# 0xMiden/miden-vm

Measured on NVIDIA H100. Metric: trace cells/sec proved, higher is better.
Workload: dtype u64

## Files before the change

### miden-vm_b200/csrc/kernels.cu

```cuda
#include "kernels.cuh"
#include "poseidon2.cuh"
#include "poseidon2_fast2.cuh"
#include "ntt2.cuh"
#include "blake3.cuh"
#include "keccak.cuh"
#include "rescue.cuh"
#include <algorithm>
#include <cstdio>

namespace mk {

static unsigned long long g_launches = 0;
unsigned long long launch_count() { return g_launches; }
void count_launch() { ++g_launches; }
void reset_launch_count() { g_launches = 0; }
#define COUNT_LAUNCH() (++g_launches)

void upload_constants() {
    cudaMemcpyToSymbol(p2::D_RC_EXT_INITIAL, p2::P2_RC_EXT_INITIAL, sizeof(u64) * 48);
    cudaMemcpyToSymbol(p2::D_RC_INTERNAL, p2::P2_RC_INTERNAL, sizeof(u64) * 22);
    cudaMemcpyToSymbol(p2::D_RC_EXT_TERMINAL, p2::P2_RC_EXT_TERMINAL, sizeof(u64) * 48);
    cudaMemcpyToSymbol(rsc::D_ARK1, rsc::RESCUE_ARK1, sizeof(u64) * 84);
    cudaMemcpyToSymbol(rsc::D_ARK2, rsc::RESCUE_ARK2, sizeof(u64) * 84);
}

#ifdef MDN_EMULATED
static inline void st_release_sys(u64* p, u64 v) { __atomic_store_n(p, v, __ATOMIC_RELEASE); }
static inline u64 ld_acquire_sys(const u64* p) { return __atomic_load_n(p, __ATOMIC_ACQUIRE); }
static constexpr long long BARRIER_TIMEOUT = 600ll * 1000000000ll;
#else
__device__ __forceinline__ void st_release_sys(u64* p, u64 v) { asm volatile("st.release.sys.global.u64 [%0], %1;" ::"l"(p), "l"(v) : "memory"); }
__device__ __forceinline__ u64 ld_acquire_sys(const u64* p) { u64 v; asm volatile("ld.acquire.sys.global.u64 %0, [%1];" : "=l"(v) : "l"(p) : "memory"); return v; }
static constexpr long long BARRIER_TIMEOUT = 30000000000ll;
#endif
__device__ __forceinline__ void push_u2(const PushDst& d, size_t idx, size_t owner_key, ulonglong2 v) {
    if (d.mode == PUSH_ALL) {
        for (u32 g = 0; g < d.world; g++) reinterpret_cast<ulonglong2*>(d.pp.p[g])[idx] = v;
    } else {
        u32 g = d.mode == PUSH_OWNER ? (u32)(owner_key >> d.owner_shift) : d.rank;
        reinterpret_cast<ulonglong2*>(d.pp.p[g])[idx] = v;
    }
}
struct BarrierArgs { PeerPtrs flags; u32 rank, world; u64 epoch; u32* err; };
__global__ void k_barrier(BarrierArgs a) {
    u32 p = threadIdx.x;
    if (p < a.world) { __threadfence_system(); st_release_sys(a.flags.p[p] + a.rank, a.epoch); }
    __syncthreads();
    if (p < a.world) {
        long long t0 = clock64();
        while (ld_acquire_sys(a.flags.p[a.rank] + p) < a.epoch) {
            if (clock64() - t0 > BARRIER_TIMEOUT) { atomicOr(a.err, 8u); break; }
#ifdef MDN_EMULATED
            emu::cpu_relax();
#endif
        }
    }
}
void launch_barrier(const PeerPtrs& flags, u32 rank, u32 world, u64 epoch, u32* err, cudaStream_t st) {
    BarrierArgs a; a.flags = flags; a.rank = rank; a.world = world; a.epoch = epoch; a.err = err;
    k_barrier<<<1, 32, 0, st>>>(a);
    COUNT_LAUNCH();
}
struct PushArgs { const u64* src; PeerPtrs dst; u32 rank, world; size_t n; };
__global__ void __launch_bounds__(256) k_push(PushArgs a) {
    size_t stride = (size_t)gridDim.x * blockDim.x, i0 = (size_t)blockIdx.x * blockDim.x + threadIdx.x;
    if ((a.n & 1) == 0 && (((size_t)a.src) & 15) == 0) {
        const ulonglong2* s2 = reinterpret_cast<const ulonglong2*>(a.src);
        for (size_t i = i0; i < a.n / 2; i += stride) {
            ulonglong2 v = s2[i];
            for (u32 g = 0; g < a.world; g++) if (g != a.rank) reinterpret_cast<ulonglong2*>(a.dst.p[g])[i] = v;
        }
    } else {
        for (size_t i = i0; i < a.n; i += stride) {
            u64 v = a.src[i];
            for (u32 g = 0; g < a.world; g++) if (g != a.rank) a.dst.p[g][i] = v;
        }
    }
}
void launch_push(const u64* src, const PeerPtrs& dst, u32 rank, u32 world, size_t n, cudaStream_t st) {
    if (!n || world <= 1) return;
    PushArgs a; a.src = src; a.dst = dst; a.rank = rank; a.world = world; a.n = n;
    unsigned blocks = (unsigned)std::min<size_t>((n / 2 + 255) / 256 + 1, 132 * 8);
    k_push<<<blocks, 256, 0, st>>>(a);
    COUNT_LAUNCH();
}

struct TransposeDst { PeerPtrs dst; PeerPtrs bad; u32 world; };
__global__ void k_transpose(const u64* __restrict__ src, TransposeDst d, u32 n_rows, u32 width, size_t col_stride, u32 row0) {
    __shared__ u64 tile[32][33];
    u32 r0 = blockIdx.x * 32, c0 = blockIdx.y * 32;
    bool any_bad = false;
    for (u32 i = threadIdx.y; i < 32; i += 8) {
        u32 r = r0 + i, c = c0 + threadIdx.x;
        if (r < n_rows && c < width) {
            u64 v = src[(size_t)r * width + c];
            any_bad |= (v >= gl::P);
            tile[i][threadIdx.x] = v;
        }
    }
    if (any_bad) for (u32 g = 0; g < d.world; g++) if (d.bad.p[g]) atomicOr(reinterpret_cast<u32*>(d.bad.p[g]), 1u);
    __syncthreads();
    for (u32 i = threadIdx.y; i < 32; i += 8) {
        u32 c = c0 + i, r = r0 + threadIdx.x;
        if (r < n_rows && c < width) {
            u64 v = tile[threadIdx.x][i];
            size_t o = (size_t)c * col_stride + row0 + r;
            for (u32 g = 0; g < d.world; g++) d.dst.p[g][o] = v;
        }
    }
}
void launch_transpose_rm_to_cm(const u64* src, u64* dst, u32 n_rows, u32 width, u32* d_bad_flag, cudaStream_t st) {
    TransposeDst d{}; d.dst.p[0] = dst; d.bad.p[0] = reinterpret_cast<u64*>(d_bad_flag); d.world = 1;
    dim3 grid((n_rows + 31) / 32, (width + 31) / 32), block(32, 8);
    k_transpose<<<grid, block, 0, st>>>(src, d, n_rows, width, (size_t)n_rows, 0u);
    COUNT_LAUNCH();
}
void launch_transpose_slice_push(const u64* src_slice, const PeerPtrs& dst_cm, const PeerPtrs& bad, u32 world, u32 row0, u32 n_rows_slice,
                                 u32 n_rows_total, u32 width, cudaStream_t st) {
    if (!n_rows_slice || !width) return;
    TransposeDst d{}; d.dst = dst_cm; d.bad = bad; d.world = world;
    dim3 grid((n_rows_slice + 31) / 32, (width + 31) / 32), block(32, 8);
    k_transpose<<<grid, block, 0, st>>>(src_slice, d, n_rows_slice, width, (size_t)n_rows_total, row0);
    COUNT_LAUNCH();
}

__global__ void __launch_bounds__(256) k_ingest_cm(const u64* __restrict__ src, u64* __restrict__ dst, size_t n, u32* bad) {
    const bool store = src != dst;
    size_t stride = (size_t)gridDim.x * blockDim.x, i0 = (size_t)blockIdx.x * blockDim.x + threadIdx.x;
    bool any_bad = false;
    if (((((size_t)src) | ((size_t)dst)) & 15) == 0) {
        const ulonglong2* s2 = reinterpret_cast<const ulonglong2*>(src);
        ulonglong2* d2 = reinterpret_cast<ulonglong2*>(dst);
        for (size_t i = i0; i < n / 2; i += stride) {
            ulonglong2 v = s2[i];
            any_bad |= (v.x >= gl::P) | (v.y >= gl::P);
            if (store) d2[i] = v;
        }
        if ((n & 1) && i0 == 0) {
            u64 v = src[n - 1];
            any_bad |= v >= gl::P;
            if (store) dst[n - 1] = v;
        }
    } else {
        for (size_t i = i0; i < n; i += stride) {
            u64 v = src[i];
            any_bad |= v >= gl::P;
            if (store) dst[i] = v;
        }
    }
    if (any_bad) atomicOr(bad, 1u);
}
void launch_ingest_cm(const u64* src_cm, u64* dst_cm, size_t n, u32* d_bad_flag, cudaStream_t st) {
    if (!n) return;
    unsigned blocks = (unsigned)std::min<size_t>((n / 2 + 255) / 256 + 1, 132 * 8);
    k_ingest_cm<<<blocks, 256, 0, st>>>(src_cm, dst_cm, n, d_bad_flag);
    COUNT_LAUNCH();
}

static constexpr int NTT_THREADS = 256;
static inline unsigned ntt_threads(u32 m, u32 log_cols, u32 log_elems) {
    u32 g = (m + log_cols >= log_elems) ? (1u << (m + log_cols - log_elems)) : 1u;
    if (g < 32) g = 32;
    if (g > 256) g = 256;
    return g;
}

__device__ __forceinline__ u64 w_pow(const u64* __restrict__ hi, const u64* __restrict__ lo, u32 lo_bits, u64 e) {
    return gl::mul(hi[e >> lo_bits], lo[e & ((1ull << lo_bits) - 1)]);
}

#define NTT_BOUNDS __launch_bounds__(NTT_THREADS)
template <int N1C, int N2C>
__global__ void NTT_BOUNDS k_intt_strided(u64* cols, size_t col_stride, NttTables T, u32 log_c) {
    extern __shared__ u64 sm[];
    ntt2::intt_strided_block<N1C, N2C>(blockIdx.x, blockIdx.y, sm, cols, col_stride, T, log_c);
}
template <int N2C>
__global__ void NTT_BOUNDS k_intt_contig(u64* cols, size_t col_stride, NttTables T) {
    extern __shared__ u64 sm[];
    ntt2::intt_contig_block<N2C>(blockIdx.x, blockIdx.y, sm, cols, col_stride, T);
}
template <int N1C, int N2C>
__global__ void NTT_BOUNDS k_fwd_contig(const FwdItem* __restrict__ items, NttTables T, PremulTables Pm) {
    extern __shared__ u64 sm[];
    ntt2::fwd_contig_block<N1C, N2C>(blockIdx.x, blockIdx.y, sm, items, T, Pm);
}
template <int N1C, int N2C>
__global__ void NTT_BOUNDS k_fwd_strided(const FwdItem* __restrict__ items, NttTables T, u32 log_c) {
    extern __shared__ u64 sm[];
    ntt2::fwd_strided_block<N1C, N2C>(blockIdx.x, blockIdx.y, sm, items, T, log_c);
}
#define NTT_SPECIALISED(X) X(8, 8) X(8, 9) X(9, 9) X(9, 10) X(10, 10) X(10, 11) X(11, 11)

template <int N1C, int N2C>
static void launch_intt_t(u64* cols, size_t col_stride, u32 n_cols, const NttTables& T, u32 log_c, cudaStream_t st) {
    u32 N1 = 1u << T.n1, N2 = 1u << T.n2, C = 1u << log_c;
    constexpr u32 LOG_E1 = N1C >= 0 ? ntt2::sched_log_elems(N1C) : 3, LOG_E2 = N2C >= 0 ? ntt2::sched_log_elems(N2C) : 3;
    if (T.n1 > 0) {
        size_t smem = ntt2::smem_words_strided(T.n1, log_c) * sizeof(u64);
        cudaFuncSetAttribute(k_intt_strided<N1C, N2C>, cudaFuncAttributeMaxDynamicSharedMemorySize, (int)smem);
        k_intt_strided<N1C, N2C><<<dim3(N2 / C, n_cols), ntt_threads(T.n1, log_c, LOG_E1), smem, st>>>(cols, col_stride, T, log_c);
        COUNT_LAUNCH();
    }
    size_t smem = ntt2::smem_words_contig_inv(T.n2) * sizeof(u64);
    k_intt_contig<N2C><<<dim3(N1, n_cols), ntt_threads(T.n2, 0, LOG_E2), smem, st>>>(cols, col_stride, T);
    COUNT_LAUNCH();
}
void launch_intt(u64* cols, size_t col_stride, u32 n_cols, const NttTables& T, cudaStream_t st) {
    u32 log_c = T.n1 >= 12 ? 0 : 12 - T.n1; if (log_c > T.n2) log_c = T.n2;
#define X(a, b) if (T.n1 == a && T.n2 == b) { launch_intt_t<a, b>(cols, col_stride, n_cols, T, log_c, st); return; }
    NTT_SPECIALISED(X)
#undef X
    launch_intt_t<-1, -1>(cols, col_stride, n_cols, T, log_c, st);
}
template <int N1C, int N2C>
static void launch_fwd_t(const FwdItem* d_items, u32 n_items, const NttTables& T, const PremulTables& Pm, u32 log_c, cudaStream_t st) {
    u32 N1 = 1u << T.n1, N2 = 1u << T.n2, C = 1u << log_c;
    constexpr u32 LOG_E1 = N1C >= 0 ? ntt2::sched_log_elems(N1C) : 3, LOG_E2 = N2C >= 0 ? ntt2::sched_log_elems(N2C) : 3;
    size_t smem = ntt2::smem_words_contig_fwd(T.n2) * sizeof(u64);
    k_fwd_contig<N1C, N2C><<<dim3(N1, n_items), ntt_threads(T.n2, 0, LOG_E2), smem, st>>>(d_items, T, Pm);
    COUNT_LAUNCH();
    if (T.n1 > 0) {
        size_t smem2 = ntt2::smem_words_strided(T.n1, log_c) * sizeof(u64);
        cudaFuncSetAttribute(k_fwd_strided<N1C, N2C>, cudaFuncAttributeMaxDynamicSharedMemorySize, (int)smem2);
        k_fwd_strided<N1C, N2C><<<dim3(N2 / C, n_items), ntt_threads(T.n1, log_c, LOG_E1), smem2, st>>>(d_items, T, log_c);
        COUNT_LAUNCH();
    }
}
void launch_fwd_ntt(const FwdItem* d_items, u32 n_items, const NttTables& T, const PremulTables& Pm, cudaStream_t st) {
    u32 log_c = T.n1 >= 12 ? 0 : 12 - T.n1; if (log_c > T.n2) log_c = T.n2;
#define X(a, b) if (T.n1 == a && T.n2 == b) { launch_fwd_t<a, b>(d_items, n_items, T, Pm, log_c, st); return; }
    NTT_SPECIALISED(X)
#undef X
    launch_fwd_t<-1, -1>(d_items, n_items, T, Pm, log_c, st);
}

static constexpr int HASH_THREADS = 128;
static constexpr int HASH_MIN_BLOCKS = 6;

enum { PERM_P2 = 0, PERM_RPO = 3, PERM_RPX = 4 };
template <int PERM>
__device__ __forceinline__ void alg_permute(u64* s) {
    if constexpr (PERM == PERM_RPO) rsc::rpo_permute(s);
    else if constexpr (PERM == PERM_RPX) rsc::rpx_permute(s);
    else p2f::permute(s);
}
#define ALG_BOUNDS(PERM) __launch_bounds__(HASH_THREADS, (PERM) == PERM_P2 ? HASH_MIN_BLOCKS : 1)
#define ALG_DISPATCH(perm, CALL) do { if ((perm) == PERM_RPO) { CALL(PERM_RPO); } else if ((perm) == PERM_RPX) { CALL(PERM_RPX); } else { CALL(PERM_P2); } } while (0)

template <int PERM>
__global__ void ALG_BOUNDS(PERM) k_leaf_hash(LeafArgs a, u32 log_n, u32 log_b, const u64* __restrict__ prev,
                                                            u32 prev_log_n, u64* __restrict__ states_out,
                                                            PushDst dig, u32 has_dig, u32 t0, u32 nt) {
    size_t L = (size_t)1 << (log_n + log_b);
    size_t idx = (size_t)blockIdx.x * blockDim.x + threadIdx.x;
    if (idx >= ((size_t)nt << log_n)) return;
    u32 t = t0 + (u32)(idx >> log_n);
    u32 r = (u32)(idx & (((size_t)1 << log_n) - 1));
    size_t pos = ((size_t)t << log_n) + r;
    u64 s[12];
    if (prev) {
        size_t Lp = (size_t)1 << (prev_log_n + log_b);
        size_t pp = ((size_t)t << prev_log_n) + (r & ((1u << prev_log_n) - 1));
#pragma unroll
        for (int k = 0; k < 12; k++) s[k] = prev[k * Lp + pp];
    } else {
#pragma unroll
        for (int k = 0; k < 12; k++) s[k] = 0;
    }
    for (int m = 0; m < a.n_mats; m++) {
        const u64* base = a.m[m].base + pos;
        u32 w = a.m[m].width;
        for (u32 c0 = 0; c0 < w; c0 += 8) {
#pragma unroll
            for (u32 k = 0; k < 8; k++) s[k] = (c0 + k < w) ? base[(size_t)(c0 + k) * L] : 0ull;
            alg_permute<PERM>(s);
        }
    }
    if (states_out) {
#pragma unroll
        for (int k = 0; k < 12; k++) states_out[k * L + pos] = glf::canon(s[k]);
    }
    if (has_dig) {
        size_t i = ((size_t)r << log_b) | t;
        push_u2(dig, 2 * i, i, make_ulonglong2(glf::canon(s[0]), glf::canon(s[1])));
        push_u2(dig, 2 * i + 1, i, make_ulonglong2(glf::canon(s[2]), glf::canon(s[3])));
    }
}
template <int PERM>
static void launch_leaf_hash_t(const LeafArgs& a, u32 log_n, u32 log_blowup, const u64* prev_states, u32 prev_log_n,
                               u64* states_out, const PushDst* dig, u32 t0, u32 nt, cudaStream_t st) {
    size_t cnt = (size_t)nt << log_n;
    unsigned blocks = (unsigned)((cnt + HASH_THREADS - 1) / HASH_THREADS);
    PushDst d = dig ? *dig : local_dst(nullptr);
    k_leaf_hash<PERM><<<blocks, HASH_THREADS, 0, st>>>(a, log_n, log_blowup, prev_states, prev_log_n, states_out, d, dig ? 1u : 0u, t0, nt);
    COUNT_LAUNCH();
}
void launch_leaf_hash(const LeafArgs& a, u32 log_n, u32 log_blowup, const u64* prev_states, u32 prev_log_n,
                      u64* states_out, const PushDst* dig, u32 t0, u32 nt, cudaStream_t st, int perm) {
#define X(PM) launch_leaf_hash_t<PM>(a, log_n, log_blowup, prev_states, prev_log_n, states_out, dig, t0, nt, st)
    ALG_DISPATCH(perm, X);
#undef X
}

template <int PERM>
__global__ void ALG_BOUNDS(PERM) k_compress(const u64* __restrict__ ch, u64* __restrict__ par, size_t n) {
    size_t i = (size_t)blockIdx.x * blockDim.x + threadIdx.x;
    if (i >= n) return;
    const ulonglong2* c = reinterpret_cast<const ulonglong2*>(ch + i * 8);
    ulonglong2 a0 = c[0], a1 = c[1], b0 = c[2], b1 = c[3];
    u64 s[12] = {a0.x, a0.y, a1.x, a1.y, b0.x, b0.y, b1.x, b1.y, 0, 0, 0, 0};
    alg_permute<PERM>(s);
    ulonglong2* d = reinterpret_cast<ulonglong2*>(par + i * 4);
    d[0] = make_ulonglong2(glf::canon(s[0]), glf::canon(s[1]));
    d[1] = make_ulonglong2(glf::canon(s[2]), glf::canon(s[3]));
}
template <int PERM>
static void launch_compress_layer_t(const u64* children, u64* parents, size_t n_parents, cudaStream_t st) {
    unsigned blocks = (unsigned)((n_parents + HASH_THREADS - 1) / HASH_THREADS);
    k_compress<PERM><<<blocks, HASH_THREADS, 0, st>>>(children, parents, n_parents);
    COUNT_LAUNCH();
}
void launch_compress_layer(const u64* children, u64* parents, size_t n_parents, cudaStream_t st, int perm) {
#define X(PM) launch_compress_layer_t<PM>(children, parents, n_parents, st)
    ALG_DISPATCH(perm, X);
#undef X
}

template <int PERM>
__global__ void __launch_bounds__(HASH_THREADS) k_fri_leaf(const u64* __restrict__ ev, size_t q, u32 la, PushDst dig, u32 log_b, u32 t0, u32 log_nt) {
    size_t idx = (size_t)blockIdx.x * blockDim.x + threadIdx.x;
    if (idx >= ((q >> log_b) << log_nt)) return;
    size_t i = ((idx >> log_nt) << log_b) | (t0 + (idx & ((1u << log_nt) - 1)));
    const ulonglong2* e = reinterpret_cast<const ulonglong2*>(ev);
    u64 s[12];
#pragma unroll
    for (int k = 0; k < 12; k++) s[k] = 0;
    u32 a = 1u << la;
    for (u32 j0 = 0; j0 < a; j0 += 4) {
#pragma unroll
        for (u32 j = 0; j < 4; j++) {
            if (j0 + j < a) {
                ulonglong2 v = e[i + (size_t)gl::bitrev32(j0 + j, la) * q];
                s[2 * j] = v.x; s[2 * j + 1] = v.y;
            } else { s[2 * j] = 0; s[2 * j + 1] = 0; }
        }
        alg_permute<PERM>(s);
    }
    push_u2(dig, 2 * i, i, make_ulonglong2(glf::canon(s[0]), glf::canon(s[1])));
    push_u2(dig, 2 * i + 1, i, make_ulonglong2(glf::canon(s[2]), glf::canon(s[3])));
}
static inline u32 log2_exact(u32 v) { u32 l = 0; while ((1u << l) < v) l++; return l; }
template <int PERM>
static void launch_fri_leaf_hash_t(const u64* evals, size_t rows, u32 log_arity, const PushDst& digests, u32 log_b, u32 t0, u32 nt, cudaStream_t st) {
    if (rows < ((size_t)1 << log_b)) { log_b = 0; t0 = 0; nt = 1; }
    size_t cnt = (rows >> log_b) * nt;
    unsigned blocks = (unsigned)((cnt + HASH_THREADS - 1) / HASH_THREADS);
    k_fri_leaf<PERM><<<blocks, HASH_THREADS, 0, st>>>(evals, rows, log_arity, digests, log_b, t0, log2_exact(nt));
    COUNT_LAUNCH();
}
void launch_fri_leaf_hash(const u64* evals, size_t rows, u32 log_arity, const PushDst& digests, u32 log_b, u32 t0, u32 nt, cudaStream_t st, int perm) {
#define X(PM) launch_fri_leaf_hash_t<PM>(evals, rows, log_arity, digests, log_b, t0, nt, st)
    ALG_DISPATCH(perm, X);
#undef X
}

__global__ void k_p2_batch(u64* st, size_t n) {
    size_t i = (size_t)blockIdx.x * blockDim.x + threadIdx.x;
    if (i >= n) return;
    u64 s[12];
#pragma unroll
    for (int k = 0; k < 12; k++) s[k] = st[i * 12 + k];
    p2f::permute(s);
#pragma unroll
    for (int k = 0; k < 12; k++) st[i * 12 + k] = glf::canon(s[k]);
}
void launch_poseidon2_batch(u64* states, size_t n, cudaStream_t st) {
    k_p2_batch<<<(unsigned)((n + 127) / 128), 128, 0, st>>>(states, n);
    COUNT_LAUNCH();
}

__global__ void __launch_bounds__(HASH_THREADS) k_leaf_hash_b3(LeafArgs a, u32 log_n, u32 log_b, const u64* __restrict__ prev, u32 prev_log_n,
                                                               u64* __restrict__ states_out, PushDst dig, u32 has_dig, u32 t0, u32 nt) {
    size_t L = (size_t)1 << (log_n + log_b);
    size_t idx = (size_t)blockIdx.x * blockDim.x + threadIdx.x;
    if (idx >= ((size_t)nt << log_n)) return;
    u32 t = t0 + (u32)(idx >> log_n);
    u32 r = (u32)(idx & (((size_t)1 << log_n) - 1));
    size_t pos = ((size_t)t << log_n) + r;
    u64 st[4] = {0, 0, 0, 0};
    if (prev) {
        size_t Lp = (size_t)1 << (prev_log_n + log_b);
        size_t pp = ((size_t)t << prev_log_n) + (r & ((1u << prev_log_n) - 1));
#pragma unroll
        for (int k = 0; k < 4; k++) st[k] = prev[k * Lp + pp];
    }
    for (int m = 0; m < a.n_mats; m++) {
        const u64* base = a.m[m].base + pos;
        u32 w = a.m[m].width;
        b3::Hasher h; h.init();
#pragma unroll
        for (int k = 0; k < 4; k++) h.push64(st[k]);
        for (u32 c = 0; c < w; c++) h.push64(base[(size_t)c * L]);
        u32 o[8];
        h.finish(o);
        b3::words_to_u64(o, st);
    }
    if (states_out) {
#pragma unroll
        for (int k = 0; k < 4; k++) states_out[k * L + pos] = st[k];
    }
    if (has_dig) {
        size_t i = ((size_t)r << log_b) | t;
        push_u2(dig, 2 * i, i, make_ulonglong2(st[0], st[1]));
        push_u2(dig, 2 * i + 1, i, make_ulonglong2(st[2], st[3]));
    }
}
void launch_leaf_hash_b3(const LeafArgs& a, u32 log_n, u32 log_blowup, const u64* prev_states, u32 prev_log_n,
                         u64* states_out, const PushDst* dig, u32 t0, u32 nt, cudaStream_t st) {
    size_t cnt = (size_t)nt << log_n;
    unsigned blocks = (unsigned)((cnt + HASH_THREADS - 1) / HASH_THREADS);
    PushDst d = dig ? *dig : local_dst(nullptr);
    k_leaf_hash_b3<<<blocks, HASH_THREADS, 0, st>>>(a, log_n, log_blowup, prev_states, prev_log_n, states_out, d, dig ? 1u : 0u, t0, nt);
    COUNT_LAUNCH();
}
__global__ void __launch_bounds__(256) k_compress_b3(const u64* __restrict__ ch, u64* __restrict__ par, size_t n) {
    size_t i = (size_t)blockIdx.x * blockDim.x + threadIdx.x;
    if (i >= n) return;
    const ulonglong2* c = reinterpret_cast<const ulonglong2*>(ch + i * 8);
    ulonglong2 a0 = c[0], a1 = c[1], b0 = c[2], b1 = c[3];
    u64 l[4] = {a0.x, a0.y, a1.x, a1.y}, r[4] = {b0.x, b0.y, b1.x, b1.y}, o[4];
    b3::compress2(l, r, o);
    ulonglong2* d = reinterpret_cast<ulonglong2*>(par + i * 4);
    d[0] = make_ulonglong2(o[0], o[1]);
    d[1] = make_ulonglong2(o[2], o[3]);
}
void launch_compress_layer_b3(const u64* children, u64* parents, size_t n_parents, cudaStream_t st) {
    k_compress_b3<<<(unsigned)((n_parents + 255) / 256), 256, 0, st>>>(children, parents, n_parents);
    COUNT_LAUNCH();
}
__global__ void __launch_bounds__(256) k_fri_leaf_b3(const u64* __restrict__ ev, size_t q, u32 la, PushDst dig, u32 log_b, u32 t0, u32 log_nt) {
    size_t idx = (size_t)blockIdx.x * blockDim.x + threadIdx.x;
    if (idx >= ((q >> log_b) << log_nt)) return;
    size_t i = ((idx >> log_nt) << log_b) | (t0 + (idx & ((1u << log_nt) - 1)));
    const ulonglong2* e = reinterpret_cast<const ulonglong2*>(ev);
    b3::Hasher h; h.init();
    for (int k = 0; k < 4; k++) h.push64(0);
    u32 a = 1u << la;
    for (u32 j = 0; j < a; j++) {
        ulonglong2 v = e[i + (size_t)gl::bitrev32(j, la) * q];
        h.push64(v.x); h.push64(v.y);
    }
    u32 o[8]; u64 d[4];
    h.finish(o);
    b3::words_to_u64(o, d);
    push_u2(dig, 2 * i, i, make_ulonglong2(d[0], d[1]));
    push_u2(dig, 2 * i + 1, i, make_ulonglong2(d[2], d[3]));
}
void launch_fri_leaf_hash_b3(const u64* evals, size_t rows, u32 log_arity, const PushDst& digests, u32 log_b, u32 t0, u32 nt, cudaStream_t st) {
    if (rows < ((size_t)1 << log_b)) { log_b = 0; t0 = 0; nt = 1; }
    size_t cnt = (rows >> log_b) * nt;
    k_fri_leaf_b3<<<(unsigned)((cnt + 255) / 256), 256, 0, st>>>(evals, rows, log_arity, digests, log_b, t0, log2_exact(nt));
    COUNT_LAUNCH();
}
__global__ void __launch_bounds__(128) k_grind_b3(const u32* __restrict__ input, u32 n_words, u64 mask, u64 start, u64 count, u64* result) {
    u64 idx = (u64)blockIdx.x * blockDim.x + threadIdx.x;
    if (idx >= count) return;
    u64 w = start + idx;
    b3::Hasher h; h.init();
    for (u32 i = 0; i < n_words; i++) h.push(input[i]);
    h.push64(w);
    u32 o[8];
    h.finish(o);
    u64 v = (u64)b3::bswap(o[7]) | ((u64)b3::bswap(o[6]) << 32);
    if ((v & mask) == 0) atomicMin(reinterpret_cast<unsigned long long*>(result), (unsigned long long)w);
}
void launch_grind_b3(const u32* d_input_words, u32 n_words, u32 bits, u64 start, u64 count, u64* d_result, cudaStream_t st) {
    u64 mask = (1ull << bits) - 1;
    k_grind_b3<<<(unsigned)((count + 127) / 128), 128, 0, st>>>(d_input_words, n_words, mask, start, count, d_result);
    COUNT_LAUNCH();
}

__global__ void __launch_bounds__(HASH_THREADS) k_leaf_hash_kk(LeafArgs a, u32 log_n, u32 log_b, const u64* __restrict__ prev, u32 prev_log_n,
                                                               u64* __restrict__ states_out, PushDst dig, u32 has_dig, u32 t0, u32 nt) {
    size_t L = (size_t)1 << (log_n + log_b);
    size_t idx = (size_t)blockIdx.x * blockDim.x + threadIdx.x;
    if (idx >= ((size_t)nt << log_n)) return;
    u32 t = t0 + (u32)(idx >> log_n);
    u32 r = (u32)(idx & (((size_t)1 << log_n) - 1));
    size_t pos = ((size_t)t << log_n) + r;
    u64 st[25];
    if (prev) {
        size_t Lp = (size_t)1 << (prev_log_n + log_b);
        size_t pp = ((size_t)t << prev_log_n) + (r & ((1u << prev_log_n) - 1));
#pragma unroll
        for (int k = 0; k < 25; k++) st[k] = prev[k * Lp + pp];
    } else {
#pragma unroll
        for (int k = 0; k < 25; k++) st[k] = 0;
    }
    for (int m = 0; m < a.n_mats; m++) {
        const u64* base = a.m[m].base + pos;
        u32 w = a.m[m].width;
        for (u32 c0 = 0; c0 < w; c0 += 17) {
#pragma unroll
            for (u32 k = 0; k < 17; k++) st[k] = (c0 + k < w) ? base[(size_t)(c0 + k) * L] : 0ull;
            kk::permute(st);
        }
    }
    if (states_out) {
#pragma unroll
        for (int k = 0; k < 25; k++) states_out[k * L + pos] = st[k];
    }
    if (has_dig) {
        size_t i = ((size_t)r << log_b) | t;
        push_u2(dig, 2 * i, i, make_ulonglong2(st[0], st[1]));
        push_u2(dig, 2 * i + 1, i, make_ulonglong2(st[2], st[3]));
    }
}
void launch_leaf_hash_kk(const LeafArgs& a, u32 log_n, u32 log_blowup, const u64* prev_states, u32 prev_log_n,
                         u64* states_out, const PushDst* dig, u32 t0, u32 nt, cudaStream_t st) {
    size_t cnt = (size_t)nt << log_n;
    unsigned blocks = (unsigned)((cnt + HASH_THREADS - 1) / HASH_THREADS);
// ... 1120 lines not shown
```

### miden-vm_b200/csrc/ntt2.cuh

```cuda
#pragma once
#include "poseidon2_fast2.cuh"
#include "kernels.cuh"
#include "tma.cuh"

namespace ntt2 {
using gl::u64;
using gl::u32;

#if defined(__CUDA_ARCH__) || defined(MDN_EMULATED)
#define NTT2_FOR(i, n) for (u32 i = threadIdx.x; i < (u32)(n); i += blockDim.x)
#define NTT2_SYNC() __syncthreads()
#else
#define NTT2_FOR(i, n) for (u32 i = 0; i < (u32)(n); i++)
#define NTT2_SYNC() ((void)0)
#endif

GL_HD u32 tile_off(u32 idx, u32 cc, u32 log_cols) {
    u32 o = (idx << log_cols) + cc;
    return log_cols ? o : o + (o >> 3);
}
GL_HD u32 tile_words(u32 m, u32 log_cols) {
    u32 n = 1u << (m + log_cols);
    return log_cols ? n + (n >> 4) : n + (n >> 3) + 1;
}
GL_HD u32 tw_off(u32 m, u32 log_cols) { return (tile_words(m, log_cols) + 1u) & ~1u; }
GL_HD size_t smem_words_contig_fwd(u32 n2) { return (size_t)tw_off(n2, 0) + ((size_t)1 << n2) + 2; }
GL_HD size_t smem_words_contig_inv(u32 n2) { return (size_t)tw_off(n2, 0) + ((size_t)1 << n2) / 2 + 4; }
GL_HD size_t smem_words_strided(u32 n1, u32 log_c) { return (size_t)tw_off(n1, log_c) + ((size_t)1 << n1) / 2 + 4; }

GL_HD u32 pad16(u32 o) { return o + (o >> 4); }
template <bool P16 = false>
GL_HD u32 chunk_off(u32 i) { return P16 ? pad16(i) : tile_off(i, 0, 0); }
template <bool P16 = false>
GL_HD void load_chunk(u64* x, const u64* src, u32 n) {
#if defined(__CUDA_ARCH__)
    if (n >= 2 && (((size_t)src) & 15) == 0) {
        const ulonglong2* s2 = reinterpret_cast<const ulonglong2*>(src);
        NTT2_FOR(i, n / 2) { ulonglong2 v = s2[i]; x[chunk_off<P16>(2 * i)] = v.x; x[chunk_off<P16>(2 * i + 1)] = v.y; }
        return;
    }
#endif
    NTT2_FOR(i, n) x[chunk_off<P16>(i)] = src[i];
}
template <bool P16 = false>
GL_HD void store_chunk_canon(u64* dst, const u64* x, u32 n) {
#if defined(__CUDA_ARCH__)
    if (n >= 2 && (((size_t)dst) & 15) == 0) {
        ulonglong2* d2 = reinterpret_cast<ulonglong2*>(dst);
        NTT2_FOR(i, n / 2) d2[i] = make_ulonglong2(glf::canon_cc(x[chunk_off<P16>(2 * i)]), glf::canon_cc(x[chunk_off<P16>(2 * i + 1)]));
        return;
    }
#endif
    NTT2_FOR(i, n) dst[i] = glf::canon_cc(x[chunk_off<P16>(i)]);
}

struct TableLoad { bool async; };
GL_HD TableLoad table_load(u64* dst, const u64* src, u32 words, u64* bar) {
#if defined(__CUDA_ARCH__)
    const u32 bytes = (words * 8u + 15u) & ~15u;
    if (words >= 64 && ((((size_t)src) | ((size_t)dst)) & 15) == 0) {
        if (threadIdx.x == 0) { tma::mbar_init(bar, 1); }
        __syncthreads();
        if (threadIdx.x == 0) { tma::expect_tx(bar, bytes); tma::bulk_g2s(dst, src, bytes, bar); }
        return TableLoad{true};
    }
#endif
    (void)bar;
    NTT2_FOR(i, words) dst[i] = src[i];
    return TableLoad{false};
}
GL_HD void table_wait(TableLoad t, u64* bar) {
#if defined(__CUDA_ARCH__)
    if (t.async) tma::wait(bar, 0);
#endif
    (void)t; (void)bar;
}

template <bool STAGED>
GL_HD u64 tw_at(const u64* tw, u32 m, u32 s, u32 j) { return STAGED ? tw[((1u << s) - 1u) + j] : tw[j << (m - 1 - s)]; }

template <int LOGR, bool STAGED, bool UNIT0>
GL_HD void dit_bfly(u64* v, const u64* tw, u32 m, u32 b, u32 lo) {
    constexpr int R = 1 << LOGR;
#pragma unroll
    for (int st = 0; st < LOGR; st++) {
#pragma unroll
        for (int k = 0; k < R; k++) {
            if (k & (1 << st)) continue;
            const u32 jj = (u32)(k & ((1 << st) - 1));
            u64 c;
            if (UNIT0 && jj == 0) c = glf::canon_cc(v[k + (1 << st)]);
            else c = glf::cmul(v[k + (1 << st)], tw_at<STAGED>(tw, m, b + st, lo + (jj << b)));
            u64 a = v[k];
            v[k] = glf::add_const(a, c);
            v[k + (1 << st)] = glf::csub(a, c);
        }
    }
}
template <int LOGR, bool STAGED, bool UNIT0>
GL_HD void dit_group(u64* x, const u64* tw, u32 m, u32 b, u32 log_cols, u32 g) {
    constexpr int R = 1 << LOGR;
    u32 cc = g & ((1u << log_cols) - 1), gg = g >> log_cols;
    u32 lo = gg & ((1u << b) - 1), hi = gg >> b;
    u32 base = (hi << (b + LOGR)) | lo;
    u64 v[R];
#pragma unroll
    for (int k = 0; k < R; k++) v[k] = x[tile_off(base + ((u32)k << b), cc, log_cols)];
    dit_bfly<LOGR, STAGED, UNIT0>(v, tw, m, b, lo);
#pragma unroll
    for (int k = 0; k < R; k++) x[tile_off(base + ((u32)k << b), cc, log_cols)] = v[k];
}
template <int LOGR, bool UNIT0>
GL_HD void dif_bfly(u64* v, const u64* tw, u32 m, u32 b, u32 lo) {
    constexpr int R = 1 << LOGR;
#pragma unroll
    for (int st = LOGR - 1; st >= 0; st--) {
#pragma unroll
        for (int k = 0; k < R; k++) {
            if (k & (1 << st)) continue;
            const u32 jj = (u32)(k & ((1 << st) - 1));
            u64 a = v[k], c = glf::canon_cc(v[k + (1 << st)]);
            v[k] = glf::add_const(a, c);
            u64 d = glf::csub(a, c);
            v[k + (1 << st)] = (UNIT0 && jj == 0) ? d : glf::mul(d, tw_at<false>(tw, m, b + st, lo + (jj << b)));
        }
    }
}
template <int LOGR, bool UNIT0>
GL_HD void dif_group(u64* x, const u64* tw, u32 m, u32 b, u32 log_cols, u32 g) {
    constexpr int R = 1 << LOGR;
    u32 cc = g & ((1u << log_cols) - 1), gg = g >> log_cols;
    u32 lo = gg & ((1u << b) - 1), hi = gg >> b;
    u32 base = (hi << (b + LOGR)) | lo;
    u64 v[R];
#pragma unroll
    for (int k = 0; k < R; k++) v[k] = x[tile_off(base + ((u32)k << b), cc, log_cols)];
    dif_bfly<LOGR, UNIT0>(v, tw, m, b, lo);
#pragma unroll
    for (int k = 0; k < R; k++) x[tile_off(base + ((u32)k << b), cc, log_cols)] = v[k];
}

template <int LOGR, bool STAGED, bool UNIT0>
GL_HD void dit_round(u64* x, const u64* tw, u32 m, u32 b, u32 log_cols) {
    NTT2_FOR(g, 1u << (m - LOGR + log_cols)) dit_group<LOGR, STAGED, UNIT0>(x, tw, m, b, log_cols, g);
    NTT2_SYNC();
}
template <int LOGR, bool UNIT0>
GL_HD void dif_round(u64* x, const u64* tw, u32 m, u32 b, u32 log_cols) {
    NTT2_FOR(g, 1u << (m - LOGR + log_cols)) dif_group<LOGR, UNIT0>(x, tw, m, b, log_cols, g);
    NTT2_SYNC();
}
template <bool STAGED>
GL_HD void smem_dit(u64* x, const u64* tw, u32 m, u32 log_cols) {
    u32 b = 0;
    while (b < m) {
        u32 left = m - b;
        if (left >= 3 && left != 4) {
            if (b == 0) dit_round<3, STAGED, !STAGED>(x, tw, m, b, log_cols); else dit_round<3, STAGED, false>(x, tw, m, b, log_cols);
            b += 3;
        } else if (left == 4 || left == 2) {
            if (b == 0) dit_round<2, STAGED, !STAGED>(x, tw, m, b, log_cols); else dit_round<2, STAGED, false>(x, tw, m, b, log_cols);
            b += 2;
        } else {
            if (b == 0) dit_round<1, STAGED, !STAGED>(x, tw, m, b, log_cols); else dit_round<1, STAGED, false>(x, tw, m, b, log_cols);
            b += 1;
        }
    }
}
GL_HD void smem_dif(u64* x, const u64* tw, u32 m, u32 log_cols) {
    u32 top = m;
    while (top > 0) {
        if (top >= 3 && top != 4) {
            if (top == 3) dif_round<3, true>(x, tw, m, 0, log_cols); else dif_round<3, false>(x, tw, m, top - 3, log_cols);
            top -= 3;
        } else if (top == 4 || top == 2) {
            if (top == 2) dif_round<2, true>(x, tw, m, 0, log_cols); else dif_round<2, false>(x, tw, m, top - 2, log_cols);
            top -= 2;
        } else {
            dif_round<1, true>(x, tw, m, 0, log_cols);
            top -= 1;
        }
    }
}

GL_HD constexpr int sched_rounds(int m) { return m == 8 ? 2 : 3; }
GL_HD constexpr int sched_radix(int m, int i) { return m == 9 ? 3 : (i < 2 && (m != 10 || i == 0)) ? 4 : 3; }
GL_HD constexpr int sched_span(int m, int i) { return i == 0 ? 0 : sched_span(m, i - 1) + sched_radix(m, i - 1); }
GL_HD constexpr int sched_log_elems(int m) { return m == 9 ? 3 : 4; }

template <int LOGR, int B, int LC>
GL_HD void tile_get(u64 (&v)[1 << LOGR], const u64* x, u32 base, u32 cc) {
#pragma unroll
    for (int k = 0; k < (1 << LOGR); k++) v[k] = x[pad16(((base + ((u32)k << B)) << LC) + cc)];
}
template <int LOGR, int B, int LC>
GL_HD void tile_put(u64* x, const u64 (&v)[1 << LOGR], u32 base, u32 cc) {
#pragma unroll
    for (int k = 0; k < (1 << LOGR); k++) x[pad16(((base + ((u32)k << B)) << LC) + cc)] = v[k];
}
template <bool STAGED, int M, int LC, int I, class Ld, class St>
GL_HD void dit_sched(u64* x, const u64* tw, TableLoad tl, u64* bar, const Ld& ld, const St& st) {
    constexpr int R = sched_radix(M, I), B = sched_span(M, I);
    constexpr bool FIRST = I == 0, LAST = I + 1 == sched_rounds(M);
    NTT2_FOR(g, 1u << (M + LC - R)) {
        const u32 cc = g & ((1u << LC) - 1), gg = g >> LC, lo = gg & ((1u << B) - 1);
        const u32 base = ((gg >> B) << (B + R)) | lo;
        u64 v[1 << R];
        if constexpr (FIRST) { ld(v, base, cc); table_wait(tl, bar); } else tile_get<R, B, LC>(v, x, base, cc);
        dit_bfly<R, STAGED, B == 0 && !STAGED>(v, tw, (u32)M, (u32)B, lo);
        if constexpr (LAST) st(v, base, cc); else tile_put<R, B, LC>(x, v, base, cc);
    }
    if constexpr (!LAST) {
        NTT2_SYNC();
        dit_sched<STAGED, M, LC, I + 1>(x, tw, tl, bar, ld, st);
    }
}
template <int M, int LC, int I, class Ld, class St>
GL_HD void dif_sched(u64* x, const u64* tw, TableLoad tl, u64* bar, const Ld& ld, const St& st) {
    constexpr int R = sched_radix(M, I), B = sched_span(M, I);
    constexpr bool FIRST = I + 1 == sched_rounds(M), LAST = I == 0;
    NTT2_FOR(g, 1u << (M + LC - R)) {
        const u32 cc = g & ((1u << LC) - 1), gg = g >> LC, lo = gg & ((1u << B) - 1);
        const u32 base = ((gg >> B) << (B + R)) | lo;
        u64 v[1 << R];
        if constexpr (FIRST) { ld(v, base, cc); table_wait(tl, bar); } else tile_get<R, B, LC>(v, x, base, cc);
        dif_bfly<R, B == 0>(v, tw, (u32)M, (u32)B, lo);
        if constexpr (LAST) st(v, base, cc); else tile_put<R, B, LC>(x, v, base, cc);
    }
    if constexpr (!LAST) {
        NTT2_SYNC();
        dif_sched<M, LC, I - 1>(x, tw, tl, bar, ld, st);
    }
}

GL_HD u64 w_pow(const u64* hi, const u64* lo, u32 lo_bits, u64 e) {
    return glf::mul(hi[e >> lo_bits], lo[e & ((1ull << lo_bits) - 1)]);
}

template <int N1C, int N2C> GL_HD constexpr int strided_log_c() { return N1C >= 12 ? 0 : (12 - N1C < N2C ? 12 - N1C : N2C); }

template <int N1C = -1, int N2C = -1>
GL_HD void intt_strided_block(u32 bx, u32 by, u64* sm, u64* cols, size_t col_stride, const mk::NttTables& T, u32 log_c_rt) {
    const u32 n1 = N1C >= 0 ? (u32)N1C : T.n1, n2 = N2C >= 0 ? (u32)N2C : T.n2;
    const u32 log_c = N1C >= 0 && N2C >= 0 ? (u32)strided_log_c<N1C, N2C>() : log_c_rt;
    u32 C = 1u << log_c, N1 = 1u << n1, N2 = 1u << n2;
    u64* x = sm; u64* tw = sm + tw_off(n1, log_c); u64* bar = tw + N1 / 2 + 2;
    u64* col = cols + (size_t)by * col_stride;
    u32 j2_0 = bx * C;
    TableLoad tl = table_load(tw, T.twi_n1, N1 / 2, bar);
    if constexpr (N1C >= 0 && N2C >= 0) {
        constexpr int LC = strided_log_c<N1C, N2C>(), NR = sched_rounds(N1C);
        constexpr int RF = sched_radix(N1C, NR - 1), BF = sched_span(N1C, NR - 1), RL = sched_radix(N1C, 0);
        static_assert(BF + RF == N1C, "the rounds cover the pass");
        if (!tl.async) NTT2_SYNC();
        auto ld = [&](u64 (&v)[1 << RF], u32 base, u32 cc) {
#pragma unroll
            for (int k = 0; k < (1 << RF); k++) v[k] = col[(size_t)(base + ((u32)k << BF)) * N2 + j2_0 + cc];
        };
        auto st = [&](u64 (&v)[1 << RL], u32 base, u32 cc) {
            const u32 j2 = j2_0 + cc;
#pragma unroll
            for (int k = 0; k < (1 << RL); k++) {
                const u32 slot = base + (u32)k;
                u64 f = w_pow(T.wi_hi, T.wi_lo, T.lo_bits, (u64)j2 * gl::bitrev32(slot, n1));
                col[(size_t)slot * N2 + j2] = glf::cmul(v[k], f);
            }
        };
        dif_sched<N1C, LC, NR - 1>(x, tw, tl, bar, ld, st);
    } else {
        NTT2_FOR(idx, N1 * C) {
            u32 j1 = idx >> log_c, cc = idx & (C - 1);
            x[tile_off(j1, cc, log_c)] = col[(size_t)j1 * N2 + j2_0 + cc];
        }
        table_wait(tl, bar);
        NTT2_SYNC();
        smem_dif(x, tw, n1, log_c);
        NTT2_FOR(idx, N1 * C) {
            u32 slot = idx >> log_c, cc = idx & (C - 1);
            u32 k1 = gl::bitrev32(slot, n1);
            u32 j2 = j2_0 + cc;
            u64 f = w_pow(T.wi_hi, T.wi_lo, T.lo_bits, (u64)j2 * k1);
            col[(size_t)slot * N2 + j2] = glf::cmul(x[tile_off(slot, cc, log_c)], f);
        }
    }
}
template <int N2C = -1>
GL_HD void intt_contig_block(u32 bx, u32 by, u64* sm, u64* cols, size_t col_stride, const mk::NttTables& T) {
    const u32 n2 = N2C >= 0 ? (u32)N2C : T.n2;
    u32 N2 = 1u << n2;
    u64* x = sm; u64* tw = sm + tw_off(n2, 0); u64* bar = tw + N2 / 2 + 2;
    u64* chunk = cols + (size_t)by * col_stride + (size_t)bx * N2;
    TableLoad tl = table_load(tw, T.twi_n2, N2 / 2, bar);
    if constexpr (N2C >= 0) {
        constexpr int NR = sched_rounds(N2C), RF = sched_radix(N2C, NR - 1), BF = sched_span(N2C, NR - 1), RL = sched_radix(N2C, 0);
        static_assert(BF + RF == N2C, "the rounds cover the pass");
        if (!tl.async) NTT2_SYNC();
        auto ld = [&](u64 (&v)[1 << RF], u32 base, u32) {
#pragma unroll
            for (int k = 0; k < (1 << RF); k++) v[k] = chunk[base + ((u32)k << BF)];
        };
        auto st = [&](u64 (&v)[1 << RL], u32 base, u32) { tile_put<RL, 0, 0>(x, v, base, 0); };
        dif_sched<N2C, 0, NR - 1>(x, tw, tl, bar, ld, st);
        NTT2_SYNC();
        store_chunk_canon<true>(chunk, x, N2);
    } else {
        load_chunk(x, chunk, N2);
        table_wait(tl, bar);
        NTT2_SYNC();
        smem_dif(x, tw, n2, 0);
        store_chunk_canon(chunk, x, N2);
    }
}
static constexpr u32 FWD_LANES = 128;
template <int N1C = -1, int N2C = -1>
GL_HD void fwd_contig_block(u32 bx, u32 by, u64* sm, const mk::FwdItem* items, const mk::NttTables& T, const mk::PremulTables& Pm) {
    const u32 n1 = N1C >= 0 ? (u32)N1C : T.n1, n2 = N2C >= 0 ? (u32)N2C : T.n2, n = N1C >= 0 && N2C >= 0 ? (u32)(N1C + N2C) : T.n;
    u32 N1 = 1u << n1, N2 = 1u << n2;
    u64* x = sm; u64* tw = sm + tw_off(n2, 0); u64* bar = tw + N2;
    mk::FwdItem it = items[by];
    u32 p_hi = bx;
    u32 j1 = gl::bitrev32(p_hi, n1);
    const u64* src = it.src + (size_t)p_hi * N2;
    u64* dst = it.dst + (size_t)p_hi * N2;
    u64 fb = Pm.tab_b[(size_t)it.base * N1 + j1];
    const u64* tc = Pm.tab_c + (size_t)it.base * N2;
    TableLoad tl = table_load(tw, tc, N2, bar);
    if constexpr (N1C >= 0 && N2C >= 0) {
        constexpr int NR = sched_rounds(N2C), RF = sched_radix(N2C, 0), RL = sched_radix(N2C, NR - 1), BL = sched_span(N2C, NR - 1);
        static_assert(BL + RL == N2C, "the rounds cover the pass");
        load_chunk<true>(x, src, N2);
        NTT2_SYNC();
        const u64 mask = ((u64)1 << n) - 1;
        const u64 step = w_pow(T.w_hi, T.w_lo, T.lo_bits, ((u64)j1 << BL) & mask);
        auto ld = [&](u64 (&v)[1 << RF], u32 base, u32) { tile_get<RF, 0, 0>(v, x, base, 0); };
        auto st = [&](u64 (&v)[1 << RL], u32 base, u32) {
            u64 f = glf::mul(fb, w_pow(T.w_hi, T.w_lo, T.lo_bits, ((u64)j1 * base) & mask));
#pragma unroll
            for (int k = 0; k < (1 << RL); k++) {
                dst[base + ((u32)k << BL)] = glf::cmul(v[k], f);
                if (k + 1 < (1 << RL)) f = glf::mul(f, step);
            }
        };
        dit_sched<true, N2C, 0, 0>(x, tw, tl, bar, ld, st);
    } else {
        load_chunk(x, src, N2);
        table_wait(tl, bar);
        NTT2_SYNC();
        smem_dit<true>(x, tw, n2, 0);
        u32 lanes = N2 < FWD_LANES ? N2 : FWD_LANES;
        NTT2_FOR(l, lanes) {
            u64 f = fb, step = 1;
            if (n1 > 0) {
                u64 mask = ((u64)1 << n) - 1;
                f = glf::mul(fb, w_pow(T.w_hi, T.w_lo, T.lo_bits, ((u64)j1 * l) & mask));
                step = w_pow(T.w_hi, T.w_lo, T.lo_bits, ((u64)j1 * lanes) & mask);
            }
            for (u32 k2 = l; k2 < N2; k2 += lanes) {
                dst[k2] = glf::cmul(x[tile_off(k2, 0, 0)], f);
                if (n1 > 0) f = glf::mul(f, step);
            }
        }
    }
}
template <int N1C = -1, int N2C = -1>
GL_HD void fwd_strided_block(u32 bx, u32 by, u64* sm, const mk::FwdItem* items, const mk::NttTables& T, u32 log_c_rt) {
    const u32 n1 = N1C >= 0 ? (u32)N1C : T.n1, n2 = N2C >= 0 ? (u32)N2C : T.n2;
    const u32 log_c = N1C >= 0 && N2C >= 0 ? (u32)strided_log_c<N1C, N2C>() : log_c_rt;
    u32 C = 1u << log_c, N1 = 1u << n1, N2 = 1u << n2;
    u64* x = sm; u64* tw = sm + tw_off(n1, log_c); u64* bar = tw + N1 / 2 + 2;
    u64* col = items[by].dst;
    u32 k2_0 = bx * C;
    TableLoad tl = table_load(tw, T.tw_n1, N1 / 2, bar);
    if constexpr (N1C >= 0 && N2C >= 0) {
        constexpr int LC = strided_log_c<N1C, N2C>(), NR = sched_rounds(N1C), RF = sched_radix(N1C, 0);
        constexpr int RL = sched_radix(N1C, NR - 1), BL = sched_span(N1C, NR - 1);
        static_assert(BL + RL == N1C, "the rounds cover the pass");
        if (!tl.async) NTT2_SYNC();
        auto ld = [&](u64 (&v)[1 << RF], u32 base, u32 cc) {
#pragma unroll
            for (int k = 0; k < (1 << RF); k++) v[k] = col[(size_t)(base + (u32)k) * N2 + k2_0 + cc];
        };
        auto st = [&](u64 (&v)[1 << RL], u32 base, u32 cc) {
#pragma unroll
            for (int k = 0; k < (1 << RL); k++) col[(size_t)(base + ((u32)k << BL)) * N2 + k2_0 + cc] = glf::canon_cc(v[k]);
        };
        dit_sched<false, N1C, LC, 0>(x, tw, tl, bar, ld, st);
    } else {
        NTT2_FOR(idx, N1 * C) {
            u32 p_hi = idx >> log_c, cc = idx & (C - 1);
            x[tile_off(p_hi, cc, log_c)] = col[(size_t)p_hi * N2 + k2_0 + cc];
        }
        table_wait(tl, bar);
        NTT2_SYNC();
        smem_dit<false>(x, tw, n1, log_c);
        NTT2_FOR(idx, N1 * C) {
            u32 k1 = idx >> log_c, cc = idx & (C - 1);
            col[(size_t)k1 * N2 + k2_0 + cc] = glf::canon_cc(x[tile_off(k1, cc, log_c)]);
        }
    }
}

}
```

Baseline: 594.7 million.

## Process two NTT chunks per block in forward contiguous pass sharing twiddle table

```diff
diff --git a/miden-vm_b200/csrc/kernels.cu b/miden-vm_b200/csrc/kernels.cu
--- a/miden-vm_b200/csrc/kernels.cu
+++ b/miden-vm_b200/csrc/kernels.cu
@@ -180,10 +180,12 @@
     extern __shared__ u64 sm[];
     ntt2::intt_contig_block<N2C>(blockIdx.x, blockIdx.y, sm, cols, col_stride, T);
 }
+template <int N1C> static constexpr int fwd_contig_lch() { return N1C >= 0 ? 1 : 0; }
+template <int N2C> static constexpr int fwd_contig_min_blocks() { return N2C < 0 ? 6 : N2C <= 10 ? 4 : 3; }
 template <int N1C, int N2C>
-__global__ void NTT_BOUNDS k_fwd_contig(const FwdItem* __restrict__ items, NttTables T, PremulTables Pm) {
+__global__ void __launch_bounds__(NTT_THREADS, fwd_contig_min_blocks<N2C>()) k_fwd_contig(const FwdItem* __restrict__ items, NttTables T, PremulTables Pm) {
     extern __shared__ u64 sm[];
-    ntt2::fwd_contig_block<N1C, N2C>(blockIdx.x, blockIdx.y, sm, items, T, Pm);
+    ntt2::fwd_contig_block<N1C, N2C, fwd_contig_lch<N1C>()>(blockIdx.x, blockIdx.y, sm, items, T, Pm);
 }
 template <int N1C, int N2C>
 __global__ void NTT_BOUNDS k_fwd_strided(const FwdItem* __restrict__ items, NttTables T, u32 log_c) {
@@ -217,8 +219,10 @@
 static void launch_fwd_t(const FwdItem* d_items, u32 n_items, const NttTables& T, const PremulTables& Pm, u32 log_c, cudaStream_t st) {
     u32 N1 = 1u << T.n1, N2 = 1u << T.n2, C = 1u << log_c;
     constexpr u32 LOG_E1 = N1C >= 0 ? ntt2::sched_log_elems(N1C) : 3, LOG_E2 = N2C >= 0 ? ntt2::sched_log_elems(N2C) : 3;
-    size_t smem = ntt2::smem_words_contig_fwd(T.n2) * sizeof(u64);
-    k_fwd_contig<N1C, N2C><<<dim3(N1, n_items), ntt_threads(T.n2, 0, LOG_E2), smem, st>>>(d_items, T, Pm);
+    constexpr u32 LCH = fwd_contig_lch<N1C>();
+    size_t smem = ntt2::smem_words_contig_fwd(T.n2, LCH) * sizeof(u64);
+    cudaFuncSetAttribute(k_fwd_contig<N1C, N2C>, cudaFuncAttributeMaxDynamicSharedMemorySize, (int)smem);
+    k_fwd_contig<N1C, N2C><<<dim3(N1 >> LCH, n_items), ntt_threads(T.n2, LCH, LOG_E2), smem, st>>>(d_items, T, Pm);
     COUNT_LAUNCH();
     if (T.n1 > 0) {
         size_t smem2 = ntt2::smem_words_strided(T.n1, log_c) * sizeof(u64);
diff --git a/miden-vm_b200/csrc/ntt2.cuh b/miden-vm_b200/csrc/ntt2.cuh
--- a/miden-vm_b200/csrc/ntt2.cuh
+++ b/miden-vm_b200/csrc/ntt2.cuh
@@ -24,7 +24,7 @@
     return log_cols ? n + (n >> 4) : n + (n >> 3) + 1;
 }
 GL_HD u32 tw_off(u32 m, u32 log_cols) { return (tile_words(m, log_cols) + 1u) & ~1u; }
-GL_HD size_t smem_words_contig_fwd(u32 n2) { return (size_t)tw_off(n2, 0) + ((size_t)1 << n2) + 2; }
+GL_HD size_t smem_words_contig_fwd(u32 n2, u32 log_ch = 0) { return (size_t)tw_off(n2, log_ch) + ((size_t)1 << n2) + 2; }
 GL_HD size_t smem_words_contig_inv(u32 n2) { return (size_t)tw_off(n2, 0) + ((size_t)1 << n2) / 2 + 4; }
 GL_HD size_t smem_words_strided(u32 n1, u32 log_c) { return (size_t)tw_off(n1, log_c) + ((size_t)1 << n1) / 2 + 4; }
 
@@ -52,6 +52,21 @@
     }
 #endif
     NTT2_FOR(i, n) dst[i] = glf::canon_cc(x[chunk_off<P16>(i)]);
+}
+template <int LC>
+GL_HD void load_chunks(u64* x, const u64* src, u32 n2) {
+    const u32 n = 1u << (n2 + LC), lo = (1u << n2) - 1;
+#if defined(__CUDA_ARCH__)
+    if ((((size_t)src) & 15) == 0) {
+        const ulonglong2* s2 = reinterpret_cast<const ulonglong2*>(src);
+        NTT2_FOR(i, n / 2) {
+            const u32 w = 2 * i, o = ((w & lo) << LC) + (w >> n2);
+            ulonglong2 v = s2[i]; x[pad16(o)] = v.x; x[pad16(o + (1u << LC))] = v.y;
+        }
+        return;
+    }
+#endif
+    NTT2_FOR(w, n) x[pad16(((w & lo) << LC) + (w >> n2))] = src[w];
 }
 
 struct TableLoad { bool async; };
@@ -312,37 +327,45 @@
     }
 }
 static constexpr u32 FWD_LANES = 128;
-template <int N1C = -1, int N2C = -1>
+template <int N1C = -1, int N2C = -1, int LCH = 0>
 GL_HD void fwd_contig_block(u32 bx, u32 by, u64* sm, const mk::FwdItem* items, const mk::NttTables& T, const mk::PremulTables& Pm) {
     const u32 n1 = N1C >= 0 ? (u32)N1C : T.n1, n2 = N2C >= 0 ? (u32)N2C : T.n2, n = N1C >= 0 && N2C >= 0 ? (u32)(N1C + N2C) : T.n;
     u32 N1 = 1u << n1, N2 = 1u << n2;
-    u64* x = sm; u64* tw = sm + tw_off(n2, 0); u64* bar = tw + N2;
+    u64* x = sm; u64* tw = sm + tw_off(n2, LCH); u64* bar = tw + N2;
     mk::FwdItem it = items[by];
-    u32 p_hi = bx;
-    u32 j1 = gl::bitrev32(p_hi, n1);
-    const u64* src = it.src + (size_t)p_hi * N2;
-    u64* dst = it.dst + (size_t)p_hi * N2;
-    u64 fb = Pm.tab_b[(size_t)it.base * N1 + j1];
     const u64* tc = Pm.tab_c + (size_t)it.base * N2;
     TableLoad tl = table_load(tw, tc, N2, bar);
     if constexpr (N1C >= 0 && N2C >= 0) {
+        static_assert(LCH == 0 || LCH == 1, "one or two chunks per block");
         constexpr int NR = sched_rounds(N2C), RF = sched_radix(N2C, 0), RL = sched_radix(N2C, NR - 1), BL = sched_span(N2C, NR - 1);
         static_assert(BL + RL == N2C, "the rounds cover the pass");
-        load_chunk<true>(x, src, N2);
+        const u32 p0 = bx << LCH;
+        load_chunks<LCH>(x, it.src + (size_t)p0 * N2, (u32)N2C);
         NTT2_SYNC();
         const u64 mask = ((u64)1 << n) - 1;
-        const u64 step = w_pow(T.w_hi, T.w_lo, T.lo_bits, ((u64)j1 << BL) & mask);
-        auto ld = [&](u64 (&v)[1 << RF], u32 base, u32) { tile_get<RF, 0, 0>(v, x, base, 0); };
-        auto st = [&](u64 (&v)[1 << RL], u32 base, u32) {
-            u64 f = glf::mul(fb, w_pow(T.w_hi, T.w_lo, T.lo_bits, ((u64)j1 * base) & mask));
+        const u32 j1a = gl::bitrev32(p0, n1), j1b = LCH ? gl::bitrev32(p0 + 1, n1) : j1a;
+        const u64 fba = Pm.tab_b[(size_t)it.base * N1 + j1a], fbb = LCH ? Pm.tab_b[(size_t)it.base * N1 + j1b] : fba;
+        const u64 stepa = w_pow(T.w_hi, T.w_lo, T.lo_bits, ((u64)j1a << BL) & mask);
+        const u64 stepb = LCH ? w_pow(T.w_hi, T.w_lo, T.lo_bits, ((u64)j1b << BL) & mask) : stepa;
+        auto ld = [&](u64 (&v)[1 << RF], u32 base, u32 cc) { tile_get<RF, 0, LCH>(v, x, base, cc); };
+        auto st = [&](u64 (&v)[1 << RL], u32 base, u32 cc) {
+            const u32 j1 = cc ? j1b : j1a;
+            const u64 step = cc ? stepb : stepa;
+            u64* dst = it.dst + (size_t)(p0 + cc) * N2;
+            u64 f = glf::mul(cc ? fbb : fba, w_pow(T.w_hi, T.w_lo, T.lo_bits, ((u64)j1 * base) & mask));
 #pragma unroll
             for (int k = 0; k < (1 << RL); k++) {
                 dst[base + ((u32)k << BL)] = glf::cmul(v[k], f);
                 if (k + 1 < (1 << RL)) f = glf::mul(f, step);
             }
         };
-        dit_sched<true, N2C, 0, 0>(x, tw, tl, bar, ld, st);
+        dit_sched<true, N2C, LCH, 0>(x, tw, tl, bar, ld, st);
     } else {
+        u32 p_hi = bx;
+        u32 j1 = gl::bitrev32(p_hi, n1);
+        const u64* src = it.src + (size_t)p_hi * N2;
+        u64* dst = it.dst + (size_t)p_hi * N2;
+        u64 fb = Pm.tab_b[(size_t)it.base * N1 + j1];
         load_chunk(x, src, N2);
         table_wait(tl, bar);
         NTT2_SYNC();
```

Measured after the change: 595.4 million (median of 6 runs). Within noise of the previous version (+0.1%).
